# m-hamza-mughal/RAG-Gesture

Measured on AMD Instinct MI355X. Metric: SMPL-X frames/sec, len150 DDIM-50 + insertion guidance; 1/2/4/8 GPU, higher is better.
Workload: dtype bf16

## Files before the change

include/rg_gesture.h:

```cpp
#ifndef RG_GESTURE_H
#define RG_GESTURE_H

#include <stdint.h>

#ifdef __cplusplus
extern "C" {
#endif

typedef struct rg_handle rg_handle;

enum rg_status {
  RG_OK = 0,
  RG_ERR_INVALID = -1,
  RG_ERR_HIP = -2,
  RG_ERR_NO_DEVICE = -3
};

#define RG_VERSION 128
int rg_version(void);
int rg_create(rg_handle** out, int device);
void rg_destroy(rg_handle* h);
const char* rg_last_error(rg_handle* h);
int rg_num_cus(rg_handle* h);

int rg_ddim_update(rg_handle* h, const float* x, const float* x0, float* x_out, int64_t n,
                   float c_recip, float c_recipm1, float c_a, float c_b, void* stream);

int rg_cfg_ddim_update(rg_handle* h, const float* out, const float* x, float* x_out, float* x0_out,
                       const float* js, int B, int T, int D, float w_c, float w_u,
                       float c_recip, float c_recipm1, float c_a, float c_b, void* stream);
int rg_cfg_ddim_update_rows(rg_handle* h, const float* out_cond, const float* out_uncond, const float* x, float* x_out,
                            float* x_out2, const float* js, int B, int T, int D, float w_c, float w_u,
                            float c_recip, float c_recipm1, float c_a, float c_b, void* stream);
// ... 315 lines not shown
                     const int* query_host, int query_len, double* out, void* stream);
int rg_partial_ratio_max_len(void);

int rg_select_top_scores(rg_handle* h, const double* score, const int* top, int n_entries, double* workspace,
                         int* cursor, int cap, int* out_idx, int* out_top, double* out_score, void* stream);
int rg_select_workspace_doubles(int n_entries);
int rg_select_top_scores_batched(rg_handle* h, const double* score, const int* top, int n_entries, int n_queries,
                                 double* workspace, int* cursor, int cap, int* out_idx, int* out_top,
                                 double* out_score, void* stream);
int rg_discourse_select_fused(rg_handle* h, const int* spk, const int* rel_off, const int* rel_sense, const int* rel_conn,
                              const double* rel_prom, int n_entries, const double* params, int n_queries, double* workspace,
                              int* cursor, int cap, int* out_idx, int* out_top, double* out_score, void* stream);

int rg_text_diag_sim(rg_handle* h, const float* q, int Lq, const float* feats, const int64_t* feat_off,
                     const int* cand, int n_cand, int dim, double* out, void* stream);

typedef struct rg_fgd_layer_args {
  const float* x;
  float* y;
  float* r;
  float* s;
  const int* clip_off;
  const int* clip_off_host;
  const int* row_ptr;
  const int* col;
  const float* w_res;
  const float* w_sc;
  const float* b_res;
  const float* b_sc;
  const float* gamma;
// ... 343 lines not shown
```

profiles/lane_timeline.py:

```python
import importlib
import os
import sys
import time

import torch

sys.path.insert(0, os.path.dirname(os.path.dirname(os.path.abspath(__file__))))
rg = importlib.import_module("rag-gesture_amd")
dev = torch.device("cuda", 0)
B = int(os.environ.get("B", "16"))
GI = [2] * 25 + [0] * 25
cfg = rg.synth.default_model_cfg(num_layers=8)
vae_cfgs = rg.synth.synth_vae_cfgs(decoder_arch="all_encoder")
database = rg.synth.SyntheticDataset(int(os.environ.get("DB", "32768")), seed=2025, device=dev, feat_device=dev)
model = rg.build_architecture(rg.synth.reference_style_model_cfg(cfg, vae_cfgs, with_retrieval=True), database=database, device=dev,
                              **__import__("json").loads(os.environ.get("MODEL_KWARGS", "{}")))
model.load_state_dict(rg.synth.synth_full_state(0, cfg, vae_cfgs))
model.eval()
if "SEQ_PAIRS" in os.environ:
    model.session_options["seq_pairs"] = bool(int(os.environ["SEQ_PAIRS"]))
if "MAX_INFLIGHT" in os.environ:
    model.max_inflight = int(os.environ["MAX_INFLIGHT"])
if "SLOTS" in os.environ:
    model.slots = int(os.environ["SLOTS"])
# ... 74 lines not shown
            t0 = time.perf_counter()
            r = fn(*a, **k)
            dt = (time.perf_counter() - t0) * 1e3
            if dt > 0.5:
                fr = [f for f in traceback.extract_stack()[:-1] if "rag-gesture_amd" in f.filename][-3:]
                blocks.append(((t0 - t_step[0]) * 1e3, dt, "%s.%s" % (getattr(owner, "__name__", owner), name),
                               " < ".join("%s:%d" % (os.path.basename(f.filename), f.lineno) for f in reversed(fr))))
            return r
        setattr(owner, name, w)
    for owner, names in ((torch.Tensor, ("cpu", "item", "tolist", "numpy", "to", "nonzero", "__bool__", "__int__", "__float__", "copy_", "__setitem__", "__getitem__", "pin_memory", "index_copy_", "index_select", "clone", "record_stream")),
                         (torch.cuda.Event, ("synchronize",)), (torch.cuda.Stream, ("synchronize",)), (torch.cuda, ("synchronize",)),
                         (torch, ("tensor", "as_tensor", "stack", "cat", "zeros", "empty", "randn"))):
        for nm in names:
            wrap(owner, nm)

if os.environ.get("TIMED_REGION"):
    K = int(os.environ["TIMED_REGION"])
    model.flush()
    torch.cuda.synchronize()
    for _ in range(K):
        one_step(sync=False)
    model.flush()
    torch.cuda.synchronize()
    one_step(trace=True, sync=False)
    for _ in range(K - 1):
        one_step(sync=False)
    model.flush()
    torch.cuda.synchronize()
    print("timed region: %d batches + flush done at %.1f ms" % (K, (time.perf_counter() - t_step[0]) * 1e3))
    for i, (key, h0, h1, e0, e1) in enumerate(log):
        if key[0] in ("cobatch", "dec", "invert", "sample", "inv", "loop") or "cob" in str(key[0]) or True:
            print("   %-44s host call %6.1f -> %6.1f ms | device %6.1f -> %6.1f ms (%.1f)" % (
                str(key)[:44], h0, h1, ev_step[0].elapsed_time(e0), ev_step[0].elapsed_time(e1), e0.elapsed_time(e1)))
    sys.exit(0)

if os.environ.get("BACK_TO_BACK"):
    one_step(trace=True, sync=False)
    marks = [len(log)]
    for _ in range(int(os.environ.get("BACK_TO_BACK", "3")) - 1):
        one_step(sync=False)
        marks.append(len(log))
    torch.cuda.synchronize()
    print("three steps back to back, all done at %.1f ms" % ((time.perf_counter() - t_step[0]) * 1e3))
    for i, (key, h0, h1, e0, e1) in enumerate(log):
# ... 7 lines not shown
```

rag-gesture_amd/csrc/rg_api.hip:

```cpp
#include "rg_common.h"

extern "C" int rg_version(void) { return RG_VERSION; }

extern "C" int rg_create(rg_handle** out, int device) {
  if (!out) return RG_ERR_INVALID;
  *out = nullptr;
  int n = 0;
  if (hipGetDeviceCount(&n) != hipSuccess || n <= 0) return RG_ERR_NO_DEVICE;
  if (device < 0 || device >= n) return RG_ERR_INVALID;
  rg_handle* h = new rg_handle();
  h->device = device;
  hipDeviceProp_t prop;
  if (hipGetDeviceProperties(&prop, device) == hipSuccess) h->num_cus = prop.multiProcessorCount;
  *out = h;
  return RG_OK;
}

extern "C" void rg_destroy(rg_handle* h) { delete h; }

extern "C" const char* rg_last_error(rg_handle* h) { return h ? h->err.c_str() : "null handle"; }

extern "C" int rg_num_cus(rg_handle* h) { return h ? h->num_cus : 0; }

namespace {
__global__ void rg_lane_form_kernel(int* state, int lane, int nlanes, int narrow_wgs, int wide_wgs, int budget) {
  if (threadIdx.x != 0) return;
  int others = 0;
  for (int l = 0; l < nlanes; ++l)
    if (l != lane) others += __hip_atomic_load(state + l * RG_LANE_STRIDE, __ATOMIC_RELAXED, __HIP_MEMORY_SCOPE_AGENT);
  const int wide = wide_wgs > narrow_wgs && others + wide_wgs <= budget;
  __hip_atomic_store(state + lane * RG_LANE_STRIDE, wide ? wide_wgs : narrow_wgs, __ATOMIC_RELAXED, __HIP_MEMORY_SCOPE_AGENT);
  __hip_atomic_store(state + lane * RG_LANE_STRIDE + 1, wide, __ATOMIC_RELAXED, __HIP_MEMORY_SCOPE_AGENT);
}
// ... 13 lines not shown
```

rag-gesture_amd/csrc/rg_common.h:

```cpp
#pragma once
#include <hip/hip_runtime.h>
#include <stdint.h>
#include <stdio.h>
#include <string>

#include "../../include/rg_gesture.h"
#include "rg_once.h"

#include <vector>

struct rg_prof_rec {
  hipEvent_t start, stop;
  int variant;
  double flops;
};

struct rg_handle {
  int device = 0;
  int num_cus = 256;
  std::string err;
  int gemm_path = 0;
  int gemm_waves = 0;
  bool profiling = false;
  std::vector<rg_prof_rec> prof;
  std::vector<hipEvent_t> ev_pool;
};

#define RG_REQUIRE(h, cond, msg)                                   \
  do {                                                             \
    if (!(cond)) {                                                 \
      if (h) (h)->err = std::string(__func__) + ": " + (msg);      \
      return RG_ERR_INVALID;                                       \
    }                                                              \
  } while (0)

#define RG_CHECK_LAUNCH(h)                                                         \
  do {                                                                             \
    hipError_t e__ = hipGetLastError();                                            \
    if (e__ != hipSuccess) {                                                       \
      if (h) (h)->err = std::string(__func__) + ": " + hipGetErrorString(e__);     \
      return RG_ERR_HIP;                                                           \
// ... 162 lines not shown
```

rag-gesture_amd/csrc/rg_retrieval.hip:

```cpp
#include "rg_common.h"

namespace {

__device__ __forceinline__ void discourse_score_value(
    const int e, const int* __restrict__ spk, const int* __restrict__ rel_off, const int* __restrict__ rel_sense,
    const int* __restrict__ rel_conn, const double* __restrict__ rel_prom, int q_sense, int q_conn,
    int q_spk, double q_prom, double& score_ret, int& top_ret) {
  const int r0 = rel_off[e], r1 = rel_off[e + 1];
  double score = 0.0;
  int top = -1;
  int first = -1, conn_hit = -1;
  for (int r = r0; r < r1; ++r) {
    if (rel_sense[r] == q_sense) {
      if (first < 0) first = r;
      if (conn_hit < 0 && q_conn >= 0 && rel_conn[r] == q_conn) conn_hit = r;
    }
  }
  if (first >= 0) {
    score += 2.0;
    top = first;
    bool chosen = false;
    if (conn_hit >= 0) {
      score += 4.0;
      top = conn_hit;
// ... 116 lines not shown
          best_r = r;
        }
        ++cnt;
      }
      if (cnt > 0) {
        const double ps = sum / (double)cnt;
        score = f32 ? (double)((float)score + (float)ps) : score + ps;
        top = best_r - r0;
      }
    }
  }
  score_out[e] = score;
  top_out[e] = top;
}

__global__ void __launch_bounds__(256) text_diag_sim_kernel(const float* __restrict__ q, int Lq,
                                                           const float* __restrict__ feats,
                                                           const int64_t* __restrict__ feat_off,
                                                           const int* __restrict__ cand, int dim,
                                                           double* __restrict__ out) {
  __shared__ double red[4];
  const int c = cand[blockIdx.x];
  const int64_t o0 = feat_off[c];
  const int Ld = (int)(feat_off[c + 1] - o0);
  const int n = Lq < Ld ? Lq : Ld;
  const int d4 = dim >> 2;
  const float4* qa = reinterpret_cast<const float4*>(q);
  const float4* fa = reinterpret_cast<const float4*>(feats + o0 * dim);
  double acc = 0.0;
  for (int i = threadIdx.x; i < n * d4; i += 256) {
    const float4 a = qa[i], b = fa[i];
    acc += (double)(a.x * b.x) + (double)(a.y * b.y) + (double)(a.z * b.z) + (double)(a.w * b.w);
  }
#pragma unroll
  for (int off = 1; off < 64; off <<= 1) acc += __shfl_xor(acc, off);
  if ((threadIdx.x & 63) == 0) red[threadIdx.x >> 6] = acc;
  __syncthreads();
  if (threadIdx.x == 0) out[blockIdx.x] = n > 0 ? ((red[0] + red[1]) + (red[2] + red[3])) / (double)n : 0.0;
}

constexpr int SEL_K = 10;
constexpr int SEL_IPT = 4;

__device__ __forceinline__ double wave_max_f64(double v) {
#pragma unroll
  for (int off = 1; off < 64; off <<= 1) {
    const double o = __shfl_xor(v, off);
    v = o > v ? o : v;
  }
  return v;
}

__device__ __forceinline__ void wave_top_rounds(double (&v)[SEL_IPT], double (&tops)[SEL_K]) {
// ... 377 lines not shown
                     rg_stream(stream), spk, rel_off, rel_sense, rel_conn, rel_prom, n_entries, params, score_out, top_out);
  RG_CHECK_LAUNCH(h);
  return RG_OK;
}

extern "C" int rg_text_diag_sim(rg_handle* h, const float* q, int Lq, const float* feats, const int64_t* feat_off,
                                const int* cand, int n_cand, int dim, double* out, void* stream) {
  RG_REQUIRE(h, q && feats && feat_off && cand && out, "null pointer");
  RG_REQUIRE(h, n_cand > 0 && Lq > 0 && dim % 4 == 0, "bad shape");
  hipLaunchKernelGGL(text_diag_sim_kernel, dim3(n_cand), dim3(256), 0, rg_stream(stream), q, Lq, feats, feat_off,
                     cand, dim, out);
  RG_CHECK_LAUNCH(h);
  return RG_OK;
}

extern "C" int rg_gesture_scores(rg_handle* h, const int* spk, const int* lab_off, const int* lab_type, const int* lab_word,
                                 const double* lab_prom, const double* word_sim, int n_entries, int q_type, int q_word,
                                 int q_spk, double spk_bonus, double q_prom, int sim_f32, double* score_out, int* top_out,
                                 void* stream) {
  RG_REQUIRE(h, spk && lab_off && lab_type && lab_word && word_sim && score_out && top_out, "null pointer");
  RG_REQUIRE(h, n_entries > 0, "empty database");
  hipLaunchKernelGGL(gesture_scores_kernel, dim3((n_entries + 255) / 256), dim3(256), 0, rg_stream(stream), spk, lab_off,
                     lab_type, lab_word, lab_prom, word_sim, n_entries, q_type, q_word, q_spk, spk_bonus, q_prom, sim_f32,
                     score_out, top_out);
  RG_CHECK_LAUNCH(h);
  return RG_OK;
}

extern "C" int rg_partial_ratio(rg_handle* h, const int* vocab, const int* vocab_len, int n_words, int stride,
                                const int* query_host, int query_len, double* out, void* stream) {
// ... 13 lines not shown
```

rag-gesture_amd/pipeline.py:

```python
import collections
import ctypes
import contextlib
import copy
import os
import time
import types

import torch
import yaml

from . import capi, denoiser, sampler, schedule as sched_mod, seqfwd, vae as vae_mod

MODELS = {}


def register_module(cls):
    MODELS[cls.__name__] = cls
    return cls


def register_with_mmcv(force=False):
    regs = []
    try:
        from mmcv.cnn import MODELS as mmcv_models
# ... 266 lines not shown
class MotionDiffusion(torch.nn.Module):

    profile_phases = False
    rotation_lanes = None
    form_lanes = None
    _cur_rot = None
    _last_state = None

    def __init__(self, model=None, loss_recon=None, loss_gen=None, loss_contact=None, loss_laplace=None,
                 diffusion_train=None, diffusion_test=None, init_cfg=None, inference_type="ddpm",
                 genloss_acceleration_weight=True, genloss_hands_weight=2, genloss_smooth=True,
                 body_part_lossweights=None, device="cuda", precision="bf16", lanes=2, sample_lanes=None, session_options=None,
                 vae_options=None, async_results=False, slots=2, max_inflight=2, cobatch_lanes="batch", base_lanes=8,
                 batch_lanes=4, lane_streams=None, calibrate_lanes=True, decode_stream=False, dynamic_forms=False, dynamic_budget=None, invert_alone_wide=True, tail_glue=True,
                 cache_exemplar_latents=True, exemplar_cache_bytes=8 << 30, skip_clip_encode=True, grouped_decode=True,
                 grouped_drain=True, grouped_chains=True, **kwargs):
        super().__init__()
        self.grouped_chains, self._parked, self._win, self._n_rot = bool(grouped_chains), [], 0, 1
        self.grouped_drain = bool(grouped_drain)
        self.grouped_decode = bool(grouped_decode)
        self.cache_exemplar_latents, self.exemplar_cache_bytes = bool(cache_exemplar_latents), int(exemplar_cache_bytes)
        self.skip_clip_encode = bool(skip_clip_encode)
        self.model = build_submodule(model, device=device, **kwargs)
        dt = dict(diffusion_test)
        self.schedule = sched_mod.Schedule(beta_scheduler=dt["beta_scheduler"], diffusion_steps=dt["diffusion_steps"],
                                           respace=dt.get("respace"))
        capi.require(dt.get("model_mean_type", "start_x") == "start_x" and dt.get("classifier_free_guidance_scale", 0) == 0,
                "unsupported argument: requires dt.get(\"model_mean_type\", \"start_x\") == \"start_x\" and dt.get(\"classifier_free_guidance_scale\", 0) == 0")
        self.inference_type = inference_type
        capi.require(inference_type in ("ddim", "ddpm"), "inference_type is 'ddim' (shipped config) or 'ddpm'")
        self.device, self.precision = torch.device(device), precision
        self.training = False
        self.session_options, self.vae_options = dict(session_options or {}), dict(vae_options or {})
        self.vae_options.setdefault("grouped_decode", self.grouped_decode)
        self._state = None
        self._sessions = {}
        self._graphs = {}
        self.use_graphs = True
# ... 981 lines not shown
```

rag-gesture_amd/retrieval.py:

```python
import copy
import ctypes
import json
import os
import re

import numpy as np
import torch

from . import capi


def _clean(s):
    return "".join([c for c in str(s) if c.isalnum() or c.isspace()])


def map_conns_to_prominence(conn_list, prominence_list):
    relevant = {}
    residual = copy.deepcopy(conn_list)
    for dp in prominence_list:
        dp_word = _clean(dp[0])
        for si, sc in enumerate(conn_list):
            if si not in relevant:
                relevant[si] = []
            if residual[si] is None:
# ... 66 lines not shown
            off.append(len(rs))
        i32 = lambda a: torch.tensor(a, dtype=torch.int32, device=self.dev)
        self.spk, self.rel_off, self.rel_sense, self.rel_conn = i32(spk), i32(off), i32(rs or [0]), i32(rc or [0])
        self.rel_prom = torch.tensor(rp or [0.0], dtype=torch.float64, device=self.dev)
        feats = [db["idx_2_text"][n][0].float() for n in self.names]
        foff = np.zeros(len(feats) + 1, dtype=np.int64)
        foff[1:] = np.cumsum([f.shape[0] for f in feats])
        self.feat_off = torch.from_numpy(foff).to(self.dev)
        self.feats = torch.cat(feats, dim=0).to(self.dev).contiguous()
        self.dim = self.feats.shape[1]
        self.n = len(self.names)
        self._score = torch.empty(self.n, dtype=torch.float64, device=self.dev)
        self._top = torch.empty(self.n, dtype=torch.int32, device=self.dev)

    fused_sweep = True

    def scores(self, sense, conn, speaker_id, q_prom):
        lib, vp = self.h.lib, ctypes.c_void_p
        s = torch.cuda.current_stream().cuda_stream
        rc = lib.rg_discourse_scores(self.h._h, vp(self.spk.data_ptr()), vp(self.rel_off.data_ptr()),
                                     vp(self.rel_sense.data_ptr()), vp(self.rel_conn.data_ptr()),
                                     vp(self.rel_prom.data_ptr()), self.n, self.sense_code.get(sense, -2),
                                     self.conn_code.get(conn, -1), int(speaker_id),
                                     ctypes.c_double(float("nan") if q_prom is None else float(q_prom)),
                                     vp(self._score.data_ptr()), vp(self._top.data_ptr()), vp(s))
        if rc != 0:
            raise capi.RgError("rg_discourse_scores failed: %s" % lib.rg_last_error(self.h._h).decode())
        return self._score.cpu().numpy(), self._top.cpu().numpy()

    def sweep_buffers(self, queries):
# ... 47 lines not shown

    def sims(self, q_feat_dev, cand):
        return self.sims_async(q_feat_dev, cand).cpu().numpy()

    def sims_async(self, q_feat_dev, cand):
        lib, vp = self.h.lib, ctypes.c_void_p
        c = to_device_async(torch.tensor(cand, dtype=torch.int32), self.dev)
        out = torch.empty(len(cand), dtype=torch.float64, device=self.dev)
        s = torch.cuda.current_stream().cuda_stream
        rc = lib.rg_text_diag_sim(self.h._h, vp(q_feat_dev.data_ptr()), q_feat_dev.shape[0], vp(self.feats.data_ptr()),
                                  vp(self.feat_off.data_ptr()), vp(c.data_ptr()), len(cand), self.dim,
                                  vp(out.data_ptr()), vp(s))
        if rc != 0:
            raise capi.RgError("rg_text_diag_sim failed: %s" % lib.rg_last_error(self.h._h).decode())
        return out


def discourse_queries(discourse, prominence, speaker_id):
    conns = [d[0] for d in discourse]
    q_prom = map_conns_to_prominence(conns, prominence)
    return [(d[1], d[0], speaker_id, None if q_prom[i] is None else q_prom[i][1]) for i, d in enumerate(discourse)]


def _cut_tiers(index, q_dev, survivor, sims):
    keep, kscore, ktop = survivor
    top = dict(zip(keep.tolist(), ktop.tolist()))
    o = np.argsort(-kscore, kind="stable")
    order, oscore = keep[o].tolist(), kscore[o].tolist()
    tiers, i, n = [], 0, 0
    while i < len(order) and n < 10:
        sc = oscore[i]
        if not sc > 0:
            break
        j = i
        while j < len(order) and oscore[j] == sc:
            j += 1
        tier = [int(e) for e in order[i:j]]
        slot = None
        if len(tier) > 1:
            slot = len(sims)
            sims.append(index.sims_async(q_dev, tier))
        tiers.append((tier, slot))
        n += len(tier)
        i = j
    return tiers, top


def _walk_tiers(tiers, sims_host):
    ranked = []
    for tier, slot in tiers:
        if slot is not None:
            tier = [tier[k] for k in np.argsort(-sims_host[slot], kind="stable")]
        ranked += tier
    return ranked[:10]


def discourse_retrieval_begin(index, discourse, prominence, speaker_id, encoded_text, survivors=None):
    pend = dict(discourse=discourse, queries=[], sims=[])
    if len(discourse) == 0:
        return pend
# ... 201 lines not shown
        return {}, {}, {}
    nq = len(query_bounds)
    q_types, q_words = [query_bounds[i][1] for i in range(nq)], [query_bounds[i][0] for i in range(nq)]
    q_prom = map_conns_to_prominence(q_words, prominence)
    proms = [None if q_prom[i] is None else q_prom[i][-1] for i in range(nq)]
    si, db_b = _gesture_ranked(gindex, [(t, w, speaker_id) for t, w in zip(q_types, q_words)], encoded_text,
                               word_similarity, 1.0, proms)
    return si, db_b, query_bounds


def _gesture_ranked(gindex, queries, encoded_text, word_similarity, spk_bonus, proms):
    base = gindex.base
    q_dev = encoded_text.to(base.dev).float().contiguous()
    survivors = gindex.sweep(queries, word_similarity, spk_bonus, proms)
    sims, cut = [], []
    for qi in range(len(queries)):
        cut.append(_cut_tiers(base, q_dev, survivors[qi], sims))
    sims_host = [t.cpu().numpy() for t in sims]
    sample_indexes, d_bounds = {}, {}
    for qi, (tiers, top) in enumerate(cut):
        ranked = _walk_tiers(tiers, sims_host)
        sample_indexes[qi] = [base.names[e] for e in ranked]
        d_bounds[qi] = {}
        for e in ranked:
            b = gindex.labels[e][int(top[e])]
            d_bounds[qi][base.names[e]] = (b["word"], b["name"], round(b["start"], 3), round(b["end"], 3))
    return sample_indexes, d_bounds


def place_exemplars(retr_indexes, retr_bounds, query_bounds, retrieval_method="discourse", fps=15, chunk=15,
                    motion_len=150):
    latent_len = motion_len // chunk
    prev_end = -1
# ... 85 lines not shown
        env.close()
        if name in ("idx_2_text", "idx_2_sense") and not d:
            return None
        out[name] = d
    return out


class RetrievalDatabase:
    CACHE_CAP = 4096
    REFERENCE_TRAINING_KEYS = frozenset(("motion_feat_dim", "output_dim", "num_layers", "num_motion_layers", "kinematic_coef",
                                         "num_heads", "ff_size", "stride", "sa_block_cfg", "ffn_cfg", "dropout"))

    def __init__(self, num_retrieval=None, topk=None, latent_dim=512, text_latent_dim=768, max_seq_len=150,
                 motion_fps=15, motion_framechunksize=15, dataset=None, metadata=None, device="cuda", word_similarity=None,
                 llm_output=None, stratified_db_creation=False, stratification_interval=15, lmdb_paths=None,
                 new_lmdb_cache=False, **_cfg):
        unknown = sorted(set(_cfg) - self.REFERENCE_TRAINING_KEYS)
        if unknown:
            raise capi.RgError("RetrievalDatabase: unknown configuration key(s) %s" % ", ".join(unknown))
        if metadata is None and not new_lmdb_cache:
            metadata = read_lmdb_dicts(lmdb_paths)
        if metadata is None:
            samples = getattr(dataset, "retrieval_samples", None)
            if samples is None:
                raise capi.RgError("RetrievalDatabase needs `metadata=`, readable LMDB caches under lmdb_paths=%r (lmdb and "
                                   "the legacy pyarrow.deserialize must be importable) or `dataset.retrieval_samples`"
                                   % (lmdb_paths,))
            metadata = build_db_dicts(samples, stratified_db_creation, stratification_interval)
        self.dataset = dataset
        self.num_retrieval, self.topk = num_retrieval or 1, topk
        self.max_seq_len, self.motion_fps, self.motion_framechunksize = max_seq_len, motion_fps, motion_framechunksize
        self.latent_dim, self.text_latent_dim = latent_dim, text_latent_dim
        self.index = DiscourseIndex(metadata, device)
        self.gesture_index = GestureTypeIndex(metadata, self.index) if "idx_2_gesture_labels" in metadata else None
        self.word_similarity = fuzzy_word_similarity if word_similarity is None else word_similarity
        self.llm_output = llm_output.get if isinstance(llm_output, LLMResponseCache) else llm_output
        self.test_indexes, self.test_dbounds, self.test_qbounds = {}, {}, {}
        self.phase_ms = None

    def retrieve(self, retr_method, text_features, discourse, prominence, speaker_id, idx=None, ready=None,
                 gesture_labels=None, text=None, text_times=None):
        if retr_method not in ("discourse", "gesture_type", "llm"):
            raise NotImplementedError("retrieval method %r (the reference's `prosody` raises too, raggesture.py:431)" % retr_method)
        if True:
            if ready is not None:
                si, db_b, qb = ready
            elif retr_method in ("gesture_type", "llm"):
                if self.gesture_index is None:
                    raise capi.RgError("%s retrieval needs idx_2_gesture_labels in the DB metadata (raggesture.py:262)" % retr_method)
                if retr_method == "gesture_type":
                    si, db_b, qb = gesture_type_retrieval(self.gesture_index, gesture_labels, speaker_id, text_features,
                                                          self.word_similarity)
                else:
                    if self.llm_output is None:
                        raise capi.RgError("llm retrieval needs `llm_output=` (an LLMResponseCache or a callable text -> answer)")
                    si, db_b, qb = llm_retrieval(self.gesture_index, text, text_times, speaker_id, prominence, text_features,
                                                 self.word_similarity, self.llm_output)
            else:
                si, db_b, qb = discourse_retrieval(self.index, discourse, prominence, speaker_id, text_features)
            self.test_indexes.setdefault(idx, {})[retr_method] = si
            self.test_dbounds.setdefault(idx, {})[retr_method] = db_b
            self.test_qbounds.setdefault(idx, {})[retr_method] = qb
            while len(self.test_indexes) > self.CACHE_CAP:
                old = next(iter(self.test_indexes))
                for d in (self.test_indexes, self.test_dbounds, self.test_qbounds):
                    d.pop(old, None)
        data = {q: [s for s in idxs if s != idx][:self.num_retrieval] for q, idxs in si.items()}
        return data, db_b, qb

    def __call__(self, *a, **k):
        return self.forward(*a, **k)

# ... 48 lines not shown
                noise=None, on_exemplars=None, search_stream=None, inputs_ready=None):
        gre = gesture_rep_encoder
        dev = torch.device(device)
        B = len(conditions["text_features"])
        chunk, L = self.motion_framechunksize, self.max_seq_len // self.motion_framechunksize
        T, D = 4 * L + 3, self.latent_dim
        tick = self._tick
        tick(None)
        import contextlib
        ctx = torch.cuda.stream(search_stream) if search_stream is not None else contextlib.nullcontext()
        if search_stream is not None and inputs_ready is not None:
            search_stream.wait_event(inputs_ready)
        with ctx:
            plans, ex = [], []
            spks = [int(v) for v in conditions["speaker_ids"][:, 0].tolist()]
            pending, queries = {}, []
            if retrieval_method == "discourse":
                for b in range(B):
                    qs = discourse_queries(conditions["discourse"][b], conditions["prominence"][b], spks[b])
                    pending[b] = (len(queries), len(qs))
                    queries += qs
            swept = self.index.collect(self.index.sweep_async(queries)) if queries else []
            order_b = sorted(pending)
            begun = [discourse_retrieval_begin(self.index, conditions["discourse"][b], conditions["prominence"][b], spks[b],
                                               conditions["text_features"][b],
                                               swept[pending[b][0]:pending[b][0] + pending[b][1]]) for b in order_b]
            sims = fetch_sims(begun)
            ready = {b: discourse_retrieval_finish(self.index, p, sm) for b, p, sm in zip(order_b, begun, sims)}
            for b in range(B):
                spk = spks[b]
                ri, rb, qb = self.retrieve(retrieval_method, conditions["text_features"][b], conditions["discourse"][b],
                                           conditions["prominence"][b], spk, idx=idx[b] if idx is not None else None,
                                           ready=ready.get(b),
                                           gesture_labels=(conditions.get("gesture_labels") or [None] * B)[b],
                                           text=self._clip_text(conditions, b),
                                           text_times=(conditions.get("text_times") or [None] * B)[b])
                plan = place_exemplars(ri, rb, qb, retrieval_method, self.motion_fps, chunk, self.max_seq_len)
                plans.append((plan, rb, qb))
                for qp, name, placed in plan:
                    ex.append((b, qp, name, placed))
        tick("retrieval.search")
        self.last_exemplars = [(b, qp, name, placed is not None) for b, qp, name, placed in ex]
        recs = [self.dataset[name] for _, _, name, _ in ex]
# ... 114 lines not shown
```

Before: 78220.

## Batch discourse exemplar search into one device call with packed survivor readback

```diff
diff --git a/include/rg_gesture.h b/include/rg_gesture.h
--- a/include/rg_gesture.h
+++ b/include/rg_gesture.h
@@ -16,7 +16,7 @@
   RG_ERR_NO_DEVICE = -3
 };
 
-#define RG_VERSION 128
+#define RG_VERSION 129
 int rg_version(void);
 int rg_create(rg_handle** out, int device);
 void rg_destroy(rg_handle* h);
@@ -362,6 +362,15 @@
 
 int rg_text_diag_sim(rg_handle* h, const float* q, int Lq, const float* feats, const int64_t* feat_off,
                      const int* cand, int n_cand, int dim, double* out, void* stream);
+int rg_text_diag_sim_many(rg_handle* h, const void* const* q_feat_host, const int* q_len_host, int n_queries,
+                          const int* pair_entry_host, const int* pair_query_host, int n_pairs, const float* feats,
+                          const int64_t* feat_off, int n_entries, int dim, double* out, void* stream);
+
+int rg_discourse_search_batch(rg_handle* h, const int* spk, const int* rel_off, const int* rel_sense, const int* rel_conn,
+                              const double* rel_prom, int n_entries, const float* feats, const int64_t* feat_off, int dim,
+                              const double* params_host, int n_queries, const void* const* q_feat_host, const int* q_len_host,
+                              int* n_ranked_host, int* entry_host, int* top_host, void* stream);
+int rg_retrieval_pack_rows(rg_handle* h, int rows);
 
 typedef struct rg_fgd_layer_args {
   const float* x;
diff --git a/profiles/lane_timeline.py b/profiles/lane_timeline.py
--- a/profiles/lane_timeline.py
+++ b/profiles/lane_timeline.py
@@ -112,6 +112,19 @@
         for nm in names:
             wrap(owner, nm)
 
+searches = []
+if os.environ.get("SEARCH"):
+    rdb = model.model.database
+    mark = [0.0]
+
+    def tick(name):
+        now = time.perf_counter()
+        if name is None:
+            mark[0] = now
+        elif name == "retrieval.search":
+            searches.append(((mark[0] - t_step[0]) * 1e3, (now - mark[0]) * 1e3))
+    rdb._tick = tick
+
 if os.environ.get("TIMED_REGION"):
     K = int(os.environ["TIMED_REGION"])
     model.flush()
@@ -120,12 +133,21 @@
         one_step(sync=False)
     model.flush()
     torch.cuda.synchronize()
+    searches.clear()
+    blocks.clear()
     one_step(trace=True, sync=False)
     for _ in range(K - 1):
         one_step(sync=False)
     model.flush()
     torch.cuda.synchronize()
     print("timed region: %d batches + flush done at %.1f ms" % (K, (time.perf_counter() - t_step[0]) * 1e3))
+    if searches:
+        d = sorted(s[1] for s in searches)
+        print("exemplar search, host wall per submission: median %.2f ms, min %.2f, max %.2f, sum %.1f ms over %d" % (
+            d[len(d) // 2], d[0], d[-1], sum(d), len(d)))
+        print("   (starts at ms: took ms) " + "  ".join("%.1f: %.2f" % s for s in searches))
+    for t0, dt, what, where in blocks:
+        print("   host blocked %6.1f -> %6.1f ms (%5.1f) in %s  %s" % (t0, t0 + dt, dt, what, where))
     for i, (key, h0, h1, e0, e1) in enumerate(log):
         if key[0] in ("cobatch", "dec", "invert", "sample", "inv", "loop") or "cob" in str(key[0]) or True:
             print("   %-44s host call %6.1f -> %6.1f ms | device %6.1f -> %6.1f ms (%.1f)" % (
diff --git a/rag-gesture_amd/csrc/rg_api.hip b/rag-gesture_amd/csrc/rg_api.hip
--- a/rag-gesture_amd/csrc/rg_api.hip
+++ b/rag-gesture_amd/csrc/rg_api.hip
@@ -16,7 +16,10 @@
   return RG_OK;
 }
 
-extern "C" void rg_destroy(rg_handle* h) { delete h; }
+extern "C" void rg_destroy(rg_handle* h) {
+  if (h) rg_retrieval_release(h);
+  delete h;
+}
 
 extern "C" const char* rg_last_error(rg_handle* h) { return h ? h->err.c_str() : "null handle"; }
 
diff --git a/rag-gesture_amd/csrc/rg_common.h b/rag-gesture_amd/csrc/rg_common.h
--- a/rag-gesture_amd/csrc/rg_common.h
+++ b/rag-gesture_amd/csrc/rg_common.h
@@ -24,7 +24,9 @@
   bool profiling = false;
   std::vector<rg_prof_rec> prof;
   std::vector<hipEvent_t> ev_pool;
+  struct rg_retrieval_state* retr = nullptr;
 };
+void rg_retrieval_release(rg_handle* h);
 
 #define RG_REQUIRE(h, cond, msg)                                   \
   do {                                                             \
diff --git a/rag-gesture_amd/csrc/rg_retrieval.hip b/rag-gesture_amd/csrc/rg_retrieval.hip
--- a/rag-gesture_amd/csrc/rg_retrieval.hip
+++ b/rag-gesture_amd/csrc/rg_retrieval.hip
@@ -1,4 +1,5 @@
 #include "rg_common.h"
+#include "rg_retrieval_host.h"
 
 namespace {
 
@@ -154,13 +155,9 @@
   top_out[e] = top;
 }
 
-__global__ void __launch_bounds__(256) text_diag_sim_kernel(const float* __restrict__ q, int Lq,
-                                                           const float* __restrict__ feats,
-                                                           const int64_t* __restrict__ feat_off,
-                                                           const int* __restrict__ cand, int dim,
-                                                           double* __restrict__ out) {
-  __shared__ double red[4];
-  const int c = cand[blockIdx.x];
+__device__ __forceinline__ void text_diag_sim_one(const float* __restrict__ q, int Lq, const float* __restrict__ feats,
+                                                  const int64_t* __restrict__ feat_off, const int c, int dim,
+                                                  double* __restrict__ out, double* red) {
   const int64_t o0 = feat_off[c];
   const int Ld = (int)(feat_off[c + 1] - o0);
   const int n = Lq < Ld ? Lq : Ld;
@@ -176,7 +173,79 @@
   for (int off = 1; off < 64; off <<= 1) acc += __shfl_xor(acc, off);
   if ((threadIdx.x & 63) == 0) red[threadIdx.x >> 6] = acc;
   __syncthreads();
-  if (threadIdx.x == 0) out[blockIdx.x] = n > 0 ? ((red[0] + red[1]) + (red[2] + red[3])) / (double)n : 0.0;
+  if (threadIdx.x == 0) *out = n > 0 ? ((red[0] + red[1]) + (red[2] + red[3])) / (double)n : 0.0;
+}
+
+__global__ void __launch_bounds__(256) text_diag_sim_kernel(const float* __restrict__ q, int Lq,
+                                                           const float* __restrict__ feats,
+                                                           const int64_t* __restrict__ feat_off,
+                                                           const int* __restrict__ cand, int dim,
+                                                           double* __restrict__ out) {
+  __shared__ double red[4];
+  text_diag_sim_one(q, Lq, feats, feat_off, cand[blockIdx.x], dim, out + blockIdx.x, red);
+}
+
+struct SimQuery {
+  const float* q;
+  int Lq, pad;
+};
+struct SimPair {
+  int entry, query;
+};
+__global__ void __launch_bounds__(256) text_diag_sim_many_kernel(const SimQuery* __restrict__ queries,
+                                                                const SimPair* __restrict__ pairs,
+                                                                const float* __restrict__ feats,
+                                                                const int64_t* __restrict__ feat_off, int dim,
+                                                                double* __restrict__ out) {
+  __shared__ double red[4];
+  const SimPair p = pairs[blockIdx.x];
+  const SimQuery sq = queries[p.query];
+  text_diag_sim_one(sq.q, sq.Lq, feats, feat_off, p.entry, dim, out + blockIdx.x, red);
+}
+
+struct alignas(16) PackRow {
+  double score;
+  int idx, top;
+};
+constexpr int PACK_BX = 4;
+
+__global__ void __launch_bounds__(256) survivor_pack_kernel(const int* __restrict__ cursor, const int* __restrict__ idx,
+                                                           const int* __restrict__ top, const double* __restrict__ score,
+                                                           int n_queries, int cap, long long rows_cap,
+                                                           int* __restrict__ counts_out, PackRow* __restrict__ rows_out) {
+  __shared__ long long red[2][4];
+  const int q = blockIdx.y;
+  long long before = 0, total = 0;
+  for (int j = threadIdx.x; j < n_queries; j += 256) {
+    int c = cursor[j];
+    c = c < cap ? c : cap;
+    total += c;
+    if (j < q) before += c;
+  }
+#pragma unroll
+  for (int off = 1; off < 64; off <<= 1) {
+    before += __shfl_xor(before, off);
+    total += __shfl_xor(total, off);
+  }
+  if ((threadIdx.x & 63) == 0) {
+    red[0][threadIdx.x >> 6] = before;
+    red[1][threadIdx.x >> 6] = total;
+  }
+  __syncthreads();
+  before = (red[0][0] + red[0][1]) + (red[0][2] + red[0][3]);
+  total = (red[1][0] + red[1][1]) + (red[1][2] + red[1][3]);
+  int cnt = cursor[q];
+  cnt = cnt < cap ? cnt : cap;
+  if (blockIdx.x == 0 && threadIdx.x == 0) counts_out[q] = cnt;
+  if (total > rows_cap) return;
+  const size_t o = (size_t)q * cap;
+  for (int i = blockIdx.x * 256 + threadIdx.x; i < cnt; i += PACK_BX * 256) {
+    PackRow r;
+    r.score = score[o + i];
+    r.idx = idx[o + i];
+    r.top = top[o + i];
+    rows_out[before + i] = r;
+  }
 }
 
 constexpr int SEL_K = 10;
@@ -584,6 +653,232 @@
   return RG_OK;
 }
 
+struct rg_twin_buf {
+  void* dev = nullptr;
+  void* host = nullptr;
+  size_t bytes = 0;
+  bool reserve(size_t want, bool with_host = true) {
+    if (want <= bytes) return true;
+    release();
+    if (hipMalloc(&dev, want) != hipSuccess) { dev = nullptr; return false; }
+    if (with_host && hipHostMalloc(&host, want, hipHostMallocDefault) != hipSuccess) { host = nullptr; release(); return false; }
+    bytes = want;
+    return true;
+  }
+  void release() {
+    if (dev) (void)hipFree(dev);
+    if (host) (void)hipHostFree(host);
+    dev = host = nullptr;
+    bytes = 0;
+  }
+};
+
+constexpr int PACK_ROWS_INITIAL = 4096;
+
+struct rg_retrieval_state {
+  rg_twin_buf sweep;
+  rg_twin_buf pack;
+  rg_twin_buf upload;
+  rg_twin_buf sims;
+  int pack_rows = PACK_ROWS_INITIAL, pack_q = 0;
+  hipEvent_t upload_used = nullptr;
+  bool upload_pending = false;
+  ~rg_retrieval_state() {
+    sweep.release(); pack.release(); upload.release(); sims.release();
+    if (upload_used) (void)hipEventDestroy(upload_used);
+  }
+};
+
+void rg_retrieval_release(rg_handle* h) {
+  delete h->retr;
+  h->retr = nullptr;
+}
+
+static rg_retrieval_state* retrieval_state(rg_handle* h) {
+  if (!h->retr) h->retr = new rg_retrieval_state();
+  return h->retr;
+}
+
+#define RG_HIP(h, call, what)                                                            \
+  do {                                                                                   \
+    hipError_t e__ = (call);                                                             \
+    if (e__ != hipSuccess) {                                                             \
+      (h)->err = std::string(__func__) + ": " + (what) + ": " + hipGetErrorString(e__);  \
+      return RG_ERR_HIP;                                                                 \
+    }                                                                                    \
+  } while (0)
+
+static size_t pack_header_bytes(int n_queries) { return ((size_t)n_queries * sizeof(int) + 15) / 16 * 16; }
+
+static int upload_stage(rg_handle* h, rg_retrieval_state* st, size_t bytes) {
+  if (st->upload_pending) {
+    RG_HIP(h, hipEventSynchronize(st->upload_used), "waiting for the previous upload's consumer");
+    st->upload_pending = false;
+  }
+  if (!st->upload_used) RG_HIP(h, hipEventCreateWithFlags(&st->upload_used, hipEventDisableTiming), "event");
+  if (!st->upload.reserve(bytes < 4096 ? 4096 : bytes * 2)) {
+    h->err = std::string(__func__) + ": cannot allocate the upload block";
+    return RG_ERR_HIP;
+  }
+  return RG_OK;
+}
+
+static int sims_many_launch(rg_handle* h, const void* const* q_feat_host, const int* q_len_host, int n_queries,
+                            const int* pair_entry_host, const int* pair_query_host, int n_pairs, const float* feats,
+                            const int64_t* feat_off, int n_entries, int dim, double* out, void* stream) {
+  for (int p = 0; p < n_pairs; ++p) {
+    const int e = pair_entry_host[p], q = pair_query_host[p];
+    RG_REQUIRE(h, e >= 0 && e < n_entries && q >= 0 && q < n_queries, "pair out of range");
+    RG_REQUIRE(h, q_feat_host[q] != nullptr && q_len_host[q] > 0, "a pair's query has no features");
+    RG_REQUIRE(h, (reinterpret_cast<uintptr_t>(q_feat_host[q]) & 15) == 0, "query features must be 16-byte aligned");
+  }
+  rg_retrieval_state* st = retrieval_state(h);
+  const size_t tab = (size_t)n_queries * sizeof(SimQuery), bytes = tab + (size_t)n_pairs * sizeof(SimPair);
+  const int rc = upload_stage(h, st, bytes);
+  if (rc != RG_OK) return rc;
+  SimQuery* tq = static_cast<SimQuery*>(st->upload.host);
+  for (int q = 0; q < n_queries; ++q) tq[q] = SimQuery{static_cast<const float*>(q_feat_host[q]), q_len_host[q], 0};
+  SimPair* tp = reinterpret_cast<SimPair*>(static_cast<char*>(st->upload.host) + tab);
+  for (int p = 0; p < n_pairs; ++p) tp[p] = SimPair{pair_entry_host[p], pair_query_host[p]};
+  hipStream_t s = rg_stream(stream);
+  RG_HIP(h, hipMemcpyAsync(st->upload.dev, st->upload.host, bytes, hipMemcpyHostToDevice, s), "upload");
+  hipLaunchKernelGGL(text_diag_sim_many_kernel, dim3(n_pairs), dim3(256), 0, s, static_cast<const SimQuery*>(st->upload.dev),
+                     reinterpret_cast<const SimPair*>(static_cast<const char*>(st->upload.dev) + tab), feats, feat_off, dim, out);
+  RG_CHECK_LAUNCH(h);
+  RG_HIP(h, hipEventRecord(st->upload_used, s), "event record");
+  st->upload_pending = true;
+  return RG_OK;
+}
+
+extern "C" int rg_text_diag_sim_many(rg_handle* h, const void* const* q_feat_host, const int* q_len_host, int n_queries,
+                                     const int* pair_entry_host, const int* pair_query_host, int n_pairs, const float* feats,
+                                     const int64_t* feat_off, int n_entries, int dim, double* out, void* stream) {
+  RG_REQUIRE(h, q_feat_host && q_len_host && pair_entry_host && pair_query_host && feats && feat_off && out, "null pointer");
+  RG_REQUIRE(h, n_queries > 0 && n_pairs > 0 && n_entries > 0 && dim > 0 && dim % 4 == 0, "bad shape");
+  return sims_many_launch(h, q_feat_host, q_len_host, n_queries, pair_entry_host, pair_query_host, n_pairs, feats, feat_off,
+                          n_entries, dim, out, stream);
+}
+
+extern "C" int rg_retrieval_pack_rows(rg_handle* h, int rows) {
+  if (!h) return 0;
+  rg_retrieval_state* st = retrieval_state(h);
+  if (rows > 0 && rows != st->pack_rows) {
+    (void)hipDeviceSynchronize();
+    st->pack.release();
+    st->pack_rows = rows;
+    st->pack_q = 0;
+  }
+  return st->pack_rows;
+}
+
+extern "C" int rg_discourse_search_batch(rg_handle* h, const int* spk, const int* rel_off, const int* rel_sense,
+                                        const int* rel_conn, const double* rel_prom, int n_entries, const float* feats,
+                                        const int64_t* feat_off, int dim, const double* params_host, int n_queries,
+                                        const void* const* q_feat_host, const int* q_len_host, int* n_ranked_host,
+                                        int* entry_host, int* top_host, void* stream) {
+  RG_REQUIRE(h, spk && rel_off && rel_sense && rel_conn && rel_prom && feats && feat_off, "null pointer");
+  RG_REQUIRE(h, params_host && q_feat_host && q_len_host && n_ranked_host && entry_host && top_host, "null pointer");
+  RG_REQUIRE(h, n_entries > 0 && n_queries > 0 && n_queries <= 65535 && dim > 0 && dim % 4 == 0, "bad shape");
+  rg_retrieval_state* st = retrieval_state(h);
+  hipStream_t s = rg_stream(stream);
+  const int Q = n_queries, cap = n_entries;
+  const size_t ws_doubles = (size_t)rg_select_workspace_doubles(n_entries);
+  const size_t o_params = 0, o_ws = o_params + (size_t)Q * 4 * 8, o_score = o_ws + (size_t)Q * ws_doubles * 8,
+               o_idx = o_score + (size_t)Q * cap * 8, o_top = o_idx + (size_t)Q * cap * 4, o_cursor = o_top + (size_t)Q * cap * 4,
+               sweep_bytes = o_cursor + (size_t)Q * 4;
+  if (!st->sweep.reserve(sweep_bytes, false)) {
+    h->err = std::string(__func__) + ": cannot allocate the sweep buffers";
+    return RG_ERR_HIP;
+  }
+  char* sw = static_cast<char*>(st->sweep.dev);
+  double* d_params = reinterpret_cast<double*>(sw + o_params);
+  double* d_ws = reinterpret_cast<double*>(sw + o_ws);
+  double* d_score = reinterpret_cast<double*>(sw + o_score);
+  int* d_idx = reinterpret_cast<int*>(sw + o_idx);
+  int* d_top = reinterpret_cast<int*>(sw + o_top);
+  int* d_cursor = reinterpret_cast<int*>(sw + o_cursor);
+  int rc = upload_stage(h, st, (size_t)Q * 4 * 8);
+  if (rc != RG_OK) return rc;
+  std::copy(params_host, params_host + (size_t)Q * 4, static_cast<double*>(st->upload.host));
+  RG_HIP(h, hipMemcpyAsync(d_params, st->upload.host, (size_t)Q * 4 * 8, hipMemcpyHostToDevice, s), "parameter upload");
+  rc = rg_discourse_select_fused(h, spk, rel_off, rel_sense, rel_conn, rel_prom, n_entries, d_params, Q, d_ws, d_cursor, cap,
+                                 d_idx, d_top, d_score, stream);
+  if (rc != RG_OK) return rc;
+  const int* counts = nullptr;
+  const PackRow* rows = nullptr;
+  for (int attempt = 0;; ++attempt) {
+    if (Q > st->pack_q) {
+      st->pack.release();
+      st->pack_q = (Q + 63) / 64 * 64;
+    }
+    const size_t head = pack_header_bytes(st->pack_q), block = head + (size_t)st->pack_rows * sizeof(PackRow);
+    if (!st->pack.reserve(block)) {
+      h->err = std::string(__func__) + ": cannot allocate the survivor block";
+      return RG_ERR_HIP;
+    }
+    hipLaunchKernelGGL(survivor_pack_kernel, dim3(PACK_BX, Q), dim3(256), 0, s, d_cursor, d_idx, d_top, d_score, Q, cap,
+                       (long long)st->pack_rows, static_cast<int*>(st->pack.dev),
+                       reinterpret_cast<PackRow*>(static_cast<char*>(st->pack.dev) + head));
+    RG_CHECK_LAUNCH(h);
+    RG_HIP(h, hipMemcpyAsync(st->pack.host, st->pack.dev, block, hipMemcpyDeviceToHost, s), "survivor read-back");
+    RG_HIP(h, hipStreamSynchronize(s), "synchronise");
+    st->upload_pending = false;
+    counts = static_cast<const int*>(st->pack.host);
+    rows = reinterpret_cast<const PackRow*>(static_cast<const char*>(st->pack.host) + head);
+    long long total = 0;
+    for (int q = 0; q < Q; ++q) {
+      RG_REQUIRE(h, counts[q] >= 0 && counts[q] <= cap, "survivor count out of range");
+      total += counts[q];
+    }
+    if (total <= st->pack_rows) break;
+    RG_REQUIRE(h, attempt == 0 && total <= 0x7fffffffll / 2, "the survivor block did not fit after it was grown");
+    const long long grown = std::max(2ll * st->pack_rows, (total + 1023) / 1024 * 1024);
+    st->pack.release();
+    st->pack_rows = (int)grown;
+  }
+  std::vector<rg_rank_cut> cuts(Q);
+  std::vector<int> pair_entry, pair_query, sidx, stop;
+  std::vector<double> sscore;
+  size_t row0 = 0;
+  for (int q = 0; q < Q; ++q) {
+    const int c = counts[q];
+    sidx.resize(c); stop.resize(c); sscore.resize(c);
+    for (int i = 0; i < c; ++i) {
+      const PackRow& r = rows[row0 + i];
+      RG_REQUIRE(h, r.idx >= 0 && r.idx < n_entries, "survivor entry out of range");
+      sidx[i] = r.idx; stop[i] = r.top; sscore[i] = r.score;
+    }
+    row0 += c;
+    rg_rank_cut_tiers(sidx.data(), stop.data(), sscore.data(), c, cuts[q]);
+    for (const auto& t : cuts[q].tiers)
+      if (t.second > 1)
+        for (int k = 0; k < t.second; ++k) {
+          pair_entry.push_back(cuts[q].entry[t.first + k]);
+          pair_query.push_back(q);
+        }
+  }
+  const int n_pairs = (int)pair_entry.size();
+  if (n_pairs > 0) {
+    if (!st->sims.reserve((size_t)n_pairs * 8 < 65536 ? 65536 : (size_t)n_pairs * 16)) {
+      h->err = std::string(__func__) + ": cannot allocate the similarity buffer";
+      return RG_ERR_HIP;
+    }
+    rc = sims_many_launch(h, q_feat_host, q_len_host, Q, pair_entry.data(), pair_query.data(), n_pairs, feats, feat_off,
+                          n_entries, dim, static_cast<double*>(st->sims.dev), stream);
+    if (rc != RG_OK) return rc;
+    RG_HIP(h, hipMemcpyAsync(st->sims.host, st->sims.dev, (size_t)n_pairs * 8, hipMemcpyDeviceToHost, s), "similarity read-back");
+    RG_HIP(h, hipStreamSynchronize(s), "synchronise");
+    st->upload_pending = false;
+  }
+  const double* sims = static_cast<const double*>(st->sims.host);
+  size_t s0 = 0;
+  for (int q = 0; q < Q; ++q) {
+    n_ranked_host[q] = rg_rank_walk(cuts[q], sims + s0, entry_host + (size_t)q * RG_RANK_MAX, top_host + (size_t)q * RG_RANK_MAX);
+    s0 += cuts[q].multi_members();
+  }
+  return RG_OK;
+}
+
 extern "C" int rg_gesture_scores(rg_handle* h, const int* spk, const int* lab_off, const int* lab_type, const int* lab_word,
                                  const double* lab_prom, const double* word_sim, int n_entries, int q_type, int q_word,
                                  int q_spk, double spk_bonus, double q_prom, int sim_f32, double* score_out, int* top_out,
diff --git a/rag-gesture_amd/csrc/rg_retrieval_host.h b/rag-gesture_amd/csrc/rg_retrieval_host.h
--- /dev/null
+++ b/rag-gesture_amd/csrc/rg_retrieval_host.h
@@ -0,0 +1,66 @@
+#pragma once
+#include <algorithm>
+#include <cmath>
+#include <numeric>
+#include <utility>
+#include <vector>
+
+constexpr int RG_RANK_MAX = 10;
+
+struct rg_rank_cut {
+  std::vector<int> entry, top;
+  std::vector<std::pair<int, int>> tiers;
+  int multi_members() const {
+    int n = 0;
+    for (const auto& t : tiers) n += t.second > 1 ? t.second : 0;
+    return n;
+  }
+};
+
+inline void rg_rank_cut_tiers(const int* idx, const int* top, const double* score, int n, rg_rank_cut& out) {
+  out.entry.clear();
+  out.top.clear();
+  out.tiers.clear();
+  std::vector<int> o(n > 0 ? n : 0);
+  std::iota(o.begin(), o.end(), 0);
+  std::sort(o.begin(), o.end(), [&](int a, int b) { return idx[a] < idx[b]; });
+  std::stable_sort(o.begin(), o.end(), [&](int a, int b) { return score[a] > score[b]; });
+  int i = 0, held = 0;
+  while (i < n && held < RG_RANK_MAX) {
+    const double sc = score[o[i]];
+    if (!(sc > 0)) break;
+    int j = i;
+    while (j < n && score[o[j]] == sc) ++j;
+    out.tiers.emplace_back((int)out.entry.size(), j - i);
+    for (int k = i; k < j; ++k) {
+      out.entry.push_back(idx[o[k]]);
+      out.top.push_back(top[o[k]]);
+    }
+    held += j - i;
+    i = j;
+  }
+}
+
+inline int rg_rank_walk(const rg_rank_cut& cut, const double* sims, int* entry_out, int* top_out) {
+  int n = 0, s0 = 0;
+  std::vector<int> o;
+  for (const auto& t : cut.tiers) {
+    const int first = t.first, len = t.second;
+    o.resize(len);
+    std::iota(o.begin(), o.end(), 0);
+    if (len > 1) {
+      const double* s = sims + s0;
+      std::stable_sort(o.begin(), o.end(), [&](int a, int b) {
+        const double x = -s[a], y = -s[b];
+        return x < y || (std::isnan(y) && !std::isnan(x));
+      });
+      s0 += len;
+    }
+    for (int k = 0; k < len && n < RG_RANK_MAX; ++k, ++n) {
+      entry_out[n] = cut.entry[first + o[k]];
+      top_out[n] = cut.top[first + o[k]];
+    }
+    if (n >= RG_RANK_MAX) break;
+  }
+  return n;
+}
diff --git a/rag-gesture_amd/pipeline.py b/rag-gesture_amd/pipeline.py
--- a/rag-gesture_amd/pipeline.py
+++ b/rag-gesture_amd/pipeline.py
@@ -304,14 +304,17 @@
                  vae_options=None, async_results=False, slots=2, max_inflight=2, cobatch_lanes="batch", base_lanes=8,
                  batch_lanes=4, lane_streams=None, calibrate_lanes=True, decode_stream=False, dynamic_forms=False, dynamic_budget=None, invert_alone_wide=True, tail_glue=True,
                  cache_exemplar_latents=True, exemplar_cache_bytes=8 << 30, skip_clip_encode=True, grouped_decode=True,
-                 grouped_drain=True, grouped_chains=True, **kwargs):
+                 grouped_drain=True, grouped_chains=True, batched_search=True, **kwargs):
         super().__init__()
+        self.batched_search = bool(batched_search)
         self.grouped_chains, self._parked, self._win, self._n_rot = bool(grouped_chains), [], 0, 1
         self.grouped_drain = bool(grouped_drain)
         self.grouped_decode = bool(grouped_decode)
         self.cache_exemplar_latents, self.exemplar_cache_bytes = bool(cache_exemplar_latents), int(exemplar_cache_bytes)
         self.skip_clip_encode = bool(skip_clip_encode)
         self.model = build_submodule(model, device=device, **kwargs)
+        if getattr(self.model, "database", None) is not None:
+            self.model.database.batched_search = self.batched_search
         dt = dict(diffusion_test)
         self.schedule = sched_mod.Schedule(beta_scheduler=dt["beta_scheduler"], diffusion_steps=dt["diffusion_steps"],
                                            respace=dt.get("respace"))
diff --git a/rag-gesture_amd/retrieval.py b/rag-gesture_amd/retrieval.py
--- a/rag-gesture_amd/retrieval.py
+++ b/rag-gesture_amd/retrieval.py
@@ -104,6 +104,7 @@
         self._top = torch.empty(self.n, dtype=torch.int32, device=self.dev)
 
     fused_sweep = True
+    batched_sims = True
 
     def scores(self, sense, conn, speaker_id, q_prom):
         lib, vp = self.h.lib, ctypes.c_void_p
@@ -181,6 +182,34 @@
         if rc != 0:
             raise capi.RgError("rg_text_diag_sim failed: %s" % lib.rg_last_error(self.h._h).decode())
         return out
+
+    def sims_many(self, q_feats, pair_entry, pair_query):
+        qp = np.array([t.data_ptr() for t in q_feats], dtype=np.uint64)
+        ql = np.array([t.shape[0] for t in q_feats], dtype=np.int32)
+        pe, pq = np.ascontiguousarray(pair_entry, dtype=np.int32), np.ascontiguousarray(pair_query, dtype=np.int32)
+        out = torch.empty(len(pe), dtype=torch.float64, device=self.dev)
+        self.h.call("text_diag_sim_many", qp.ctypes.data, ql.ctypes.data, len(q_feats), pe.ctypes.data, pq.ctypes.data, len(pe),
+                    self.feats, self.feat_off, self.n, self.dim, out)
+        return out
+
+    def search_batch(self, queries, q_feats):
+        Q = len(queries)
+        if Q == 0:
+            return []
+        nan = float("nan")
+        params = np.array([[float(self.sense_code.get(sense, -2)), float(self.conn_code.get(conn, -1)), float(int(spk)),
+                            nan if q_prom is None else float(q_prom)] for sense, conn, spk, q_prom in queries], dtype=np.float64)
+        qp = np.array([t.data_ptr() for t in q_feats], dtype=np.uint64)
+        ql = np.array([t.shape[0] for t in q_feats], dtype=np.int32)
+        n_ranked, entry, top = np.zeros(Q, dtype=np.int32), np.zeros((Q, 10), dtype=np.int32), np.zeros((Q, 10), dtype=np.int32)
+        self.h.call("discourse_search_batch", self.spk, self.rel_off, self.rel_sense, self.rel_conn, self.rel_prom, self.n,
+                    self.feats, self.feat_off, self.dim, params.ctypes.data, Q, qp.ctypes.data, ql.ctypes.data,
+                    n_ranked.ctypes.data, entry.ctypes.data, top.ctypes.data)
+        entry, top = entry.tolist(), top.tolist()
+        return [(entry[q][:k], top[q][:k]) for q, k in enumerate(n_ranked.tolist())]
+
+    def pack_rows(self, rows=0):
+        return int(self.h.lib.rg_retrieval_pack_rows(self.h._h, int(rows)))
 
 
 def discourse_queries(discourse, prominence, speaker_id):
@@ -211,6 +240,13 @@
         n += len(tier)
         i = j
     return tiers, top
+
+
+class _TierList:
+
+    @staticmethod
+    def sims_async(q_dev, cand):
+        return np.asarray(cand, dtype=np.int32)
 
 
 def _walk_tiers(tiers, sims_host):
@@ -442,9 +478,18 @@
     q_dev = encoded_text.to(base.dev).float().contiguous()
     survivors = gindex.sweep(queries, word_similarity, spk_bonus, proms)
     sims, cut = [], []
-    for qi in range(len(queries)):
-        cut.append(_cut_tiers(base, q_dev, survivors[qi], sims))
-    sims_host = [t.cpu().numpy() for t in sims]
+    if base.batched_sims:
+        tiers = _TierList()
+        for qi in range(len(queries)):
+            cut.append(_cut_tiers(tiers, q_dev, survivors[qi], sims))
+        sims_host = []
+        if sims:
+            flat = base.sims_many([q_dev], np.concatenate(sims), np.zeros(sum(len(t) for t in sims), dtype=np.int32)).cpu().numpy()
+            sims_host = np.split(flat, np.cumsum([len(t) for t in sims])[:-1])
+    else:
+        for qi in range(len(queries)):
+            cut.append(_cut_tiers(base, q_dev, survivors[qi], sims))
+        sims_host = [t.cpu().numpy() for t in sims]
     sample_indexes, d_bounds = {}, {}
     for qi, (tiers, top) in enumerate(cut):
         ranked = _walk_tiers(tiers, sims_host)
@@ -560,7 +605,7 @@
     def __init__(self, num_retrieval=None, topk=None, latent_dim=512, text_latent_dim=768, max_seq_len=150,
                  motion_fps=15, motion_framechunksize=15, dataset=None, metadata=None, device="cuda", word_similarity=None,
                  llm_output=None, stratified_db_creation=False, stratification_interval=15, lmdb_paths=None,
-                 new_lmdb_cache=False, **_cfg):
+                 new_lmdb_cache=False, batched_search=True, **_cfg):
         unknown = sorted(set(_cfg) - self.REFERENCE_TRAINING_KEYS)
         if unknown:
             raise capi.RgError("RetrievalDatabase: unknown configuration key(s) %s" % ", ".join(unknown))
@@ -583,6 +628,42 @@
         self.llm_output = llm_output.get if isinstance(llm_output, LLMResponseCache) else llm_output
         self.test_indexes, self.test_dbounds, self.test_qbounds = {}, {}, {}
         self.phase_ms = None
+        self.batched_search = batched_search
+
+    @property
+    def batched_search(self):
+        return self.index.batched_sims
+
+    @batched_search.setter
+    def batched_search(self, on):
+        self.index.batched_sims = bool(on)
+
+    def _search_discourse_batch(self, conditions, spks, B):
+        index = self.index
+        queries, feats, owner = [], [], []
+        for b in range(B):
+            discourse = conditions["discourse"][b]
+            if len(discourse) == 0:
+                continue
+            q_dev = conditions["text_features"][b].to(index.dev).float().contiguous()
+            qs = discourse_queries(discourse, conditions["prominence"][b], spks[b])
+            queries += qs
+            feats += [q_dev] * len(qs)
+            owner += [b] * len(qs)
+        ranked = index.search_batch(queries, feats)
+        ready = {b: ({}, {}, {}) for b in range(B)}
+        for b in set(owner):
+            ready[b] = ({}, {}, {i: (d[0].lower(), d[1], d[6], d[7]) for i, d in enumerate(conditions["discourse"][b])})
+        qi_of = {}
+        for b, (entries, tops) in zip(owner, ranked):
+            qi = qi_of[b] = qi_of.get(b, -1) + 1
+            sample_indexes, d_bounds, _ = ready[b]
+            sample_indexes[qi] = [index.names[e] for e in entries]
+            d_bounds[qi] = {}
+            for e, t in zip(entries, tops):
+                bd = index.db["idx_2_discbounds"][index.names[e]][t]
+                d_bounds[qi][index.names[e]] = (bd[1], bd[0], round(bd[4], 3), round(bd[5], 3))
+        return ready
 
     def retrieve(self, retr_method, text_features, discourse, prominence, speaker_id, idx=None, ready=None,
                  gesture_labels=None, text=None, text_times=None):
@@ -602,6 +683,9 @@
                         raise capi.RgError("llm retrieval needs `llm_output=` (an LLMResponseCache or a callable text -> answer)")
                     si, db_b, qb = llm_retrieval(self.gesture_index, text, text_times, speaker_id, prominence, text_features,
                                                  self.word_similarity, self.llm_output)
+            elif self.batched_search:
+                si, db_b, qb = self._search_discourse_batch(dict(discourse=[discourse], prominence=[prominence],
+                                                                 text_features=[text_features]), [speaker_id], 1)[0]
             else:
                 si, db_b, qb = discourse_retrieval(self.index, discourse, prominence, speaker_id, text_features)
             self.test_indexes.setdefault(idx, {})[retr_method] = si
@@ -680,19 +764,22 @@
         with ctx:
             plans, ex = [], []
             spks = [int(v) for v in conditions["speaker_ids"][:, 0].tolist()]
-            pending, queries = {}, []
-            if retrieval_method == "discourse":
-                for b in range(B):
-                    qs = discourse_queries(conditions["discourse"][b], conditions["prominence"][b], spks[b])
-                    pending[b] = (len(queries), len(qs))
-                    queries += qs
-            swept = self.index.collect(self.index.sweep_async(queries)) if queries else []
-            order_b = sorted(pending)
-            begun = [discourse_retrieval_begin(self.index, conditions["discourse"][b], conditions["prominence"][b], spks[b],
-                                               conditions["text_features"][b],
-                                               swept[pending[b][0]:pending[b][0] + pending[b][1]]) for b in order_b]
-            sims = fetch_sims(begun)
-            ready = {b: discourse_retrieval_finish(self.index, p, sm) for b, p, sm in zip(order_b, begun, sims)}
+            if retrieval_method == "discourse" and self.batched_search:
+                ready = self._search_discourse_batch(conditions, spks, B)
+            else:
+                pending, queries = {}, []
+                if retrieval_method == "discourse":
+                    for b in range(B):
+                        qs = discourse_queries(conditions["discourse"][b], conditions["prominence"][b], spks[b])
+                        pending[b] = (len(queries), len(qs))
+                        queries += qs
+                swept = self.index.collect(self.index.sweep_async(queries)) if queries else []
+                order_b = sorted(pending)
+                begun = [discourse_retrieval_begin(self.index, conditions["discourse"][b], conditions["prominence"][b], spks[b],
+                                                   conditions["text_features"][b],
+                                                   swept[pending[b][0]:pending[b][0] + pending[b][1]]) for b in order_b]
+                sims = fetch_sims(begun)
+                ready = {b: discourse_retrieval_finish(self.index, p, sm) for b, p, sm in zip(order_b, begun, sims)}
             for b in range(B):
                 spk = spks[b]
                 ri, rb, qb = self.retrieve(retrieval_method, conditions["text_features"][b], conditions["discourse"][b],
```

New measurement: 81440, median of 6. 1.04x the previous value.
